# inksci/TRPO

Hardware: AMD Instinct MI355X
Metric: TRPO updates/sec (10-iter CG + linesearch) at N states; FVP GB/s vs HBM peak (higher is better)
Workload: dtype fp32 (f16x3 split); 1 GPU; C4: 8M states, obs 128, 256x256 tanh MLP, 18 actions; full update = discount+standardise+pg+10 CG+shs FVP+line search+final losses; n_states=8000000, obs_dim=128, n_actions=18, num_params=103442, cg_iters=10, parallelism=dp1 (row shards, RCCL all-reduce of [P] FVP/grad + loss scalars)

## Files before the change

trpo_amd/csrc/kernels.h:

```cpp
#pragma once
#include <hip/hip_runtime.h>
#include <cstdint>

namespace trpo {

struct Options {
  int split_mfma;
  int split_wg;
  int chain;
  int split_f16;
  int split_min_k;
  int graphs;
  int tail;
  int fused;
  int low_seg;
  int planes;
  int rbwd0;
  int hbwd2;
  int head_fwd;
  int splits;
  int pg_splits;
  int ls_fused;
  int cg_fuse_reduce;
  int cg_p_img;
  int rfwd01;
  int fwd01;
  int rh1_planes;
  int rbwd0_bdma;
};

constexpr int kAmaxSub = 256, kAmaxStride = 32, kAmaxSlot = kAmaxSub * kAmaxStride;

__host__ __device__ inline int f16_scale_exp(float m) {
  if (!(m > 0.0f) || !(m < 3.0e38f)) return 0;
  int q = 0;
  (void)frexpf(m, &q);
  int e = 12 - q;
  return e < -100 ? -100 : (e > 100 ? 100 : e);
}
extern Options g_options;
int* option_slot(const char* name);

struct GemmSeg {
  const float* A;
  const float* B;
  int lda, ldb, K;
  const uint16_t* B3 = nullptr;
  int ldk = 0, plane = 0;
  const unsigned* amaxA = nullptr;
  const unsigned* amaxB = nullptr;
  const uint16_t* Ah = nullptr;
  const uint16_t* Al = nullptr;
  int ldp = 0, mpad = 0;
  const int* eAp = nullptr;
  const uint16_t* Bb = nullptr;
};

enum class RowEpi : int {
  kTanh = 0,
  kRHidden = 1,
  kPrepBwd = 2,
// ... 600 lines not shown
```

trpo_amd/csrc/options.cpp:

```cpp
#include "kernels.h"

#include <cstdlib>
#include <cstring>

namespace trpo {
namespace {

struct OptionRow {
  const char* name;
  const char* env;
  int Options::*field;
  int dflt;
};
constexpr OptionRow kOptionRows[] = {
    {"split_mfma", "TRPO_SPLIT_MFMA", &Options::split_mfma, 5},
    {"split_wg", "TRPO_SPLIT_WG", &Options::split_wg, 1},
    {"chain", "TRPO_CHAIN", &Options::chain, 1},
    {"split_f16", "TRPO_SPLIT_F16", &Options::split_f16, 1},
    {"split_min_k", "TRPO_SPLIT_MIN_K", &Options::split_min_k, 0},
    {"graphs", "TRPO_GRAPHS", &Options::graphs, 1},
    {"tail", "TRPO_TAIL", &Options::tail, 1},
    {"fused", "TRPO_FUSED", &Options::fused, 3},
    {"low_seg", "TRPO_LOW_SEG", &Options::low_seg, 14},
    {"planes", "TRPO_PLANES", &Options::planes, 1},
    {"rbwd0", "TRPO_RBWD0", &Options::rbwd0, 1},
    {"hbwd2", "TRPO_HBWD2", &Options::hbwd2, 2},
    {"head_fwd", "TRPO_HEAD_FWD", &Options::head_fwd, 1},
    {"splits", "TRPO_SPLITS", &Options::splits, 0},
    {"pg_splits", "TRPO_PG_SPLITS", &Options::pg_splits, 0},
    {"ls_fused", "TRPO_LS_FUSED", &Options::ls_fused, 1},
    {"cg_fuse_reduce", "TRPO_CG_FUSE_REDUCE", &Options::cg_fuse_reduce, 1},
    {"cg_p_img", "TRPO_CG_P_IMG", &Options::cg_p_img, 1},
    {"rfwd01", "TRPO_RFWD01", &Options::rfwd01, 1},
    {"fwd01", "TRPO_FWD01", &Options::fwd01, 1},
    {"rh1_planes", "TRPO_RH1_PLANES", &Options::rh1_planes, 1},
    {"rbwd0_bdma", "TRPO_RBWD0_BDMA", &Options::rbwd0_bdma, 1},
};
static_assert(sizeof kOptionRows / sizeof kOptionRows[0] == sizeof(Options) / sizeof(int),
              "every field of Options needs a row");

Options options_from_env() {
  Options o{};
  for (const OptionRow& r : kOptionRows) {
    const char* e = std::getenv(r.env);
    o.*r.field = e ? std::atoi(e) : r.dflt;
  }
  return o;
}

}

Options g_options = options_from_env();

int* option_slot(const char* name) {
  for (const OptionRow& r : kOptionRows)
    if (!std::strcmp(name, r.name)) return &(g_options.*r.field);
  return nullptr;
}

}
```

trpo_amd/csrc/rfwd.hip:

```cpp
#include "chain_common.h"

#include <stdexcept>
#include <type_traits>

namespace trpo {
namespace {

#ifndef RF_SGB
#define RF_SGB 1
#endif
#ifndef RF_ILV
#define RF_ILV 1
#endif
#ifndef RF_HOIST
#define RF_HOIST 0
#endif
#ifndef RF_HEAD
#define RF_HEAD 3
#endif
#ifndef RF_CSB
#define RF_CSB 1
#endif
#ifndef RF_ABL
#define RF_ABL 0
#endif

constexpr int kRfUnits = 2048;
constexpr int kRfChunks = 24;
constexpr int kRfLd = 256;
constexpr int kRfTile = 128, kRfWaves = 4;

__global__ void __launch_bounds__(256) rfwd01_img_kernel(const float* __restrict__ theta, const float* __restrict__ v,
                                                         int64_t offV0, int64_t offW1, int obs,
                                                         const unsigned* am_v0, const unsigned* am_w1,
                                                         const unsigned* am_v1, uint16_t* __restrict__ img,
                                                         const int* skip) {
  if (skip && *skip) return;
  const int eV0 = amax_exp(am_v0), eW = amax_exp(am_w1), eV = amax_exp(am_v1);
  const int gid = blockIdx.x * 256 + threadIdx.x;
  const int t = gid / 2560, rem = gid % 2560;
  if (t >= 8) return;
  float x[8];
  u32x4* dst;
  int plane_units;
  float sc;
  if (rem < 512) {
    const int f = rem >> 4, u = rem & 15, ks = u >> 1, h = u & 1;
#pragma unroll
    for (int q = 0; q < 8; ++q) {
      const int k = 16 * ks + 8 * h + q;
      x[q] = k < obs ? v[offV0 + (int64_t)k * 256 + 32 * t + f] : 0.0f;
    }
    sc = __builtin_ldexpf(1.0f, eV0);
    dst = reinterpret_cast<u32x4*>(img) + (size_t)(3 * t) * kRfUnits + f * 16 + (u ^ (f & 15));
    plane_units = 512;
  } else {
    const int b = rem - 512, nh = b >> 10, m = (b >> 9) & 1, r = (b >> 2) & 127, u = b & 3, uu = u >> 1, h = u & 1;
    const float* src = m ? v : theta;
#pragma unroll
    for (int q = 0; q < 8; ++q) {
      const int k = 32 * t + 16 * uu + 4 * h + 8 * (q >> 2) + (q & 3);
      x[q] = src[offW1 + (int64_t)k * 256 + 128 * nh + r];
    }
    sc = __builtin_ldexpf(1.0f, m ? eV : eW);
    dst = reinterpret_cast<u32x4*>(img) + (size_t)(3 * t + 1 + nh) * kRfUnits + m * 1024 + r * 4 +
          (u ^ ((r >> 2) & 3));
    plane_units = 512;
  }
  f16x8 hi, lo;
  split8(x, sc, hi, lo);
  dst[0] = __builtin_bit_cast(u32x4, hi);
  dst[plane_units] = __builtin_bit_cast(u32x4, lo);
}

__device__ __forceinline__ void rf_dma16(__amdgpu_buffer_rsrc_t rsrc, unsigned voff, unsigned soff, unsigned lds) {
  unsigned keep;
  asm volatile("s_mov_b32 %0, m0\n\ts_mov_b32 m0, %3\n\ts_nop 0\n\tbuffer_load_dwordx4 %1, %2, 0 offen lds\n\t"
               "s_mov_b32 m0, %0"
               : "=&s"(keep)
               : "v"(voff + soff), "s"(rsrc), "s"(lds));
}

template <int KS0, bool PL>
__global__ void __launch_bounds__(kRfWaves * 64, 1) rfwd01_kernel(const Rfwd01Args a) {
  static_assert(!RF_ILV || KS0 == 8, "interleaved DMA: one instruction per k-step of phase A");
  __shared__ u32x4 q0[kRfUnits], q1[kRfUnits], q2[kRfUnits], q3[kRfUnits];
  __shared__ float cvec[2][256];
  __shared__ float red[3][16];
  __shared__ int pex[kRfWaves][32];
  if (a.skip && *a.skip) return;
  const int tid = threadIdx.x, lane = tid & 63, s = lane & 31, h = lane >> 5;
  const int wv = __builtin_amdgcn_readfirstlane(tid >> 6);
  const int eX = __builtin_amdgcn_readfirstlane(*a.eX);
  const int eV0 = __builtin_amdgcn_readfirstlane(amax_exp(a.am_v0));
  const int eW = __builtin_amdgcn_readfirstlane(amax_exp(a.am_w1));
  const int eV = __builtin_amdgcn_readfirstlane(amax_exp(a.am_v1));
  const float uA = __builtin_ldexpf(1.0f, -(eX + eV0));
  const int64_t ntiles = (a.n + kRfTile - 1) / kRfTile;
  const __amdgpu_buffer_rsrc_t rimg =
      __builtin_amdgcn_make_buffer_rsrc((void*)a.img, 0, kRfChunks * kRfUnits * 16, 0x00020000);
  const __amdgpu_buffer_rsrc_t rxh = __builtin_amdgcn_make_buffer_rsrc((void*)a.Xh, 0, 0x7ffffff0, 0x00020000);
  const __amdgpu_buffer_rsrc_t rxl = __builtin_amdgcn_make_buffer_rsrc((void*)a.Xl, 0, 0x7ffffff0, 0x00020000);
  for (int i = tid; i < 256; i += kRfWaves * 64) {
    cvec[0][i] = a.c0[i];
    cvec[1][i] = a.c1[i];
  }
  float nv0 = 0.0f, mc0 = 0.0f;
  if constexpr (RF_CSB) {
    float q = 0.0f;
    for (int k = 0; k < a.obs; ++k) {
      const float x = a.V0[(int64_t)k * 256 + tid];
      q = fmaf(x, x, q);
    }
    float m1 = max32_dpp(sqrtf(q)), m2 = max32_dpp(fabsf(a.c0[tid]));
    m1 = fmaxf(m1, __shfl_xor(m1, 32));
    m2 = fmaxf(m2, __shfl_xor(m2, 32));
    if (lane == 0) {
      red[0][wv] = m1;
      red[1][wv] = m2;
    }
    __syncthreads();
    nv0 = fmaxf(fmaxf(red[0][0], red[0][1]), fmaxf(red[0][2], red[0][3]));
    mc0 = fmaxf(fmaxf(red[1][0], red[1][1]), fmaxf(red[1][2], red[1][3]));
    __syncthreads();
  }
  int eR = 0;
  if constexpr (PL) {
    static_assert(RF_CSB, "the planes' exponent comes from the bound");
    const float bnd = sqrtf((float)a.obs) * __builtin_ldexpf(1.0f, 12 - eX) * nv0 * 1.01f + mc0;
    eR = __builtin_amdgcn_readfirstlane(f16_scale_exp(bnd));
    if (blockIdx.x == 0 && tid == 0) *a.e_rh1 = eR;
// ... 23 lines not shown
#pragma unroll
    for (int i = 0; i < 8; ++i) dma_one(A, c, sl, r0w, i);
  };
  using kA = std::true_type;
  using kB = std::false_type;
  auto arrive = [&](bool far, bool first_a0) __attribute__((always_inline)) {
    __builtin_amdgcn_sched_barrier(0);
    if (far) asm volatile("s_waitcnt vmcnt(63)" ::: "memory");
    else if (first_a0 || (RF_ABL & 8) != 0) asm volatile("s_waitcnt vmcnt(16)" ::: "memory");
    else asm volatile("s_waitcnt vmcnt(20)" ::: "memory");
    lds_barrier();
  };
  const unsigned xlane = (unsigned)(s * 32 + 8 * h) * 2u;
  auto xload = [&](int64_t row0, f16x8 (&x)[KS0][2]) __attribute__((always_inline)) {
    if constexpr ((RF_ABL & 16) != 0) {
#pragma unroll
      for (int ks = 0; ks < KS0; ++ks) {
        unsigned u = (unsigned)row0 + ks;
        asm volatile("" : "+v"(u));
        x[ks][0] = x[ks][1] = __builtin_bit_cast(f16x8, u32x4{u, u, u, u});
      }
      return;
    }
#pragma unroll
    for (int ks = 0; ks < KS0; ++ks) {
      const int so = (int)((((unsigned)(ks >> 1) * (unsigned)a.x_mpad + (unsigned)row0) * 32u + 16u * (ks & 1)) * 2u);
      x[ks][0] = __builtin_bit_cast(f16x8, __builtin_amdgcn_raw_buffer_load_b128(rxh, xlane, so, 0));
      x[ks][1] = __builtin_bit_cast(f16x8, __builtin_amdgcn_raw_buffer_load_b128(rxl, xlane, so, 0));
    }
  };
  const unsigned hlane = PL ? (unsigned)((s >> 1) * kPairLd + 16 * (s & 1) + 4 * h) * 4u
                            : (unsigned)(s * kRfLd + 4 * h) * 4u;

  f16x8 xt[KS0][2];
  xload((int64_t)blockIdx.x * kRfTile + wv * 32, xt);
  __builtin_amdgcn_s_waitcnt(0x0f70);
  {
    const int64_t r0f = (int64_t)blockIdx.x * kRfTile + wv * 32;
    dma(kA{}, 0, 0, r0f);
    dma(kB{}, 1, 1, r0f);
    dma(kB{}, 2, 2, r0f);
  }

  float mR = 0.0f, mZ = 0.0f;
  for (int64_t tile = blockIdx.x; tile < ntiles; tile += gridDim.x) {
    const bool first = tile == (int64_t)blockIdx.x;
    const int64_t r0 = tile * kRfTile + wv * 32;
    const int64_t r0n = r0 + (int64_t)gridDim.x * kRfTile;
    const int rows = rows_of(r0);
    const __amdgpu_buffer_rsrc_t rrh =
        __builtin_amdgcn_make_buffer_rsrc((void*)(a.RH1 + r0 * kRfLd), 0, PL ? 0 : rows * kRfLd * 4, 0x00020000);
    f32x16 acc[8];
#pragma unroll
    for (int i = 0; i < 8; ++i) acc[i] = f32x16{};
    int Ps = 0;
    if constexpr (RF_CSB) {
      float q = 0.0f;
#pragma unroll
      for (int ks = 0; ks < KS0; ++ks) {
        const f16x8 x8 = xt[ks][0];
        q = __builtin_amdgcn_fdot2(__builtin_shufflevector(x8, x8, 0, 1), __builtin_shufflevector(x8, x8, 0, 1), q, false);
        q = __builtin_amdgcn_fdot2(__builtin_shufflevector(x8, x8, 2, 3), __builtin_shufflevector(x8, x8, 2, 3), q, false);
        q = __builtin_amdgcn_fdot2(__builtin_shufflevector(x8, x8, 4, 5), __builtin_shufflevector(x8, x8, 4, 5), q, false);
        q = __builtin_amdgcn_fdot2(__builtin_shufflevector(x8, x8, 6, 7), __builtin_shufflevector(x8, x8, 6, 7), q, false);
      }
      q = xadd_f<true>(q);
      const float bnd = __builtin_ldexpf(sqrtf(q), -eX) * nv0 * 1.01f + mc0;
      Ps = min(bnd > 0.0f ? f16_scale_exp(bnd) + eW : 1000, f16_scale_exp(1.0f) + eV);
    }
    int* px = pex[wv];
#pragma unroll 1
    for (int tq = 0; tq < 2; ++tq) {
#pragma unroll
      for (int tt = 0; tt < 4; ++tt) {
        const int t = 4 * tq + tt;
        const int cA = 3 * t, sA = (3 * tt) % 4;
        const bool far = t == 0 && !first;
// ... 140 lines not shown
            if (RF_SGB && (RF_ABL & 3) == 0 && k + 1 < 8) {
              __builtin_amdgcn_sched_group_barrier(0x100, 4, 0);
              __builtin_amdgcn_sched_group_barrier(0x008, 6, 0);
            }
          }
          __builtin_amdgcn_sched_barrier(0);
        }
      }
    }
    xload(r0n < a.x_mpad ? r0n : 0, xt);
    if (h == 0) px[s] = Ps;
    __builtin_amdgcn_wave_barrier();
    __builtin_amdgcn_fence(__ATOMIC_SEQ_CST, "wavefront");
    float un[16];
#pragma unroll
    for (int r = 0; r < 16; ++r) un[r] = __builtin_ldexpf(1.0f, -px[8 * (r >> 2) + 4 * h + (r & 3)]);
    __builtin_amdgcn_wave_barrier();
    const __amdgpu_buffer_rsrc_t rz =
        __builtin_amdgcn_make_buffer_rsrc((void*)(a.RZ2 + r0 * kRfLd), 0, rows * kRfLd * 4, 0x00020000);
    const unsigned zlane = (unsigned)(4 * h * kRfLd + s) * 4u;
#pragma unroll
    for (int tn = 0; tn < 8; ++tn) {
      const float cn = cvec[1][32 * tn + s];
#pragma unroll
      for (int r = 0; r < 16; ++r) {
        const float o = acc[tn][r] * un[r] + cn;
        mZ = fmaxf(mZ, fabsf(o));
        if constexpr ((RF_ABL & 8) == 0)
          __builtin_amdgcn_raw_buffer_store_b32(__builtin_bit_cast(unsigned, o), rz, zlane,
                                                ((8 * (r >> 2) + (r & 3)) * kRfLd + 32 * tn) * 4, 0);
      }
    }
  }
  asm volatile("s_waitcnt vmcnt(0)" ::: "memory");
  if constexpr (PL) {
    if ((a.n & 1) != 0 && (int64_t)blockIdx.x == (ntiles - 1) % (int64_t)gridDim.x) {
      __syncthreads();
      int col = threadIdx.x;
      asm volatile("" : "+v"(col));
      unsigned short* const p = reinterpret_cast<unsigned short*>(a.RH1 + (a.n >> 1) * kPairLd + col) + 1;
      p[0] = 0;
      p[2 * pair_plane_dwords(a.n)] = 0;
    }
  }
  amax_commit3<true>(a.am_rh1, mR, a.am_rz2, mZ, nullptr, 0.0f, red);
}


constexpr int kFwChunks = 16;

__global__ void __launch_bounds__(256) fwd01_img_kernel(const float* __restrict__ th, int64_t offW0, int64_t offW1,
                                                        int obs, const unsigned* am_w0, const unsigned* am_w1,
                                                        uint16_t* __restrict__ img) {
  const int eW0 = amax_exp(am_w0), eW1 = amax_exp(am_w1);
  const int gid = blockIdx.x * 256 + threadIdx.x;
  const int t = gid / 1536, rem = gid % 1536;
  if (t >= 8) return;
  float x[8];
  u32x4* dst;
  int plane_units;
  float sc;
  if (rem < 512) {
    const int f = rem >> 4, u = rem & 15, ks = u >> 1, h = u & 1;
#pragma unroll
    for (int q = 0; q < 8; ++q) {
      const int k = 16 * ks + 8 * h + q;
      x[q] = k < obs ? th[offW0 + (int64_t)k * 256 + 32 * t + f] : 0.0f;
    }
    sc = __builtin_ldexpf(1.0f, eW0);
    dst = reinterpret_cast<u32x4*>(img) + (size_t)(2 * t) * kRfUnits + f * 16 + (u ^ (f & 15));
    plane_units = 512;
  } else {
    const int b = rem - 512, r = b >> 2, u = b & 3, uu = u >> 1, h = u & 1;
#pragma unroll
    for (int q = 0; q < 8; ++q) {
      const int k = 32 * t + 16 * uu + 4 * h + 8 * (q >> 2) + (q & 3);
      x[q] = th[offW1 + (int64_t)k * 256 + r];
    }
    sc = __builtin_ldexpf(1.0f, eW1);
    dst = reinterpret_cast<u32x4*>(img) + (size_t)(2 * t + 1) * kRfUnits + r * 4 + (u ^ ((r >> 2) & 3));
    plane_units = 1024;
  }
  f16x8 hi, lo;
  split8(x, sc, hi, lo);
  dst[0] = __builtin_bit_cast(u32x4, hi);
  dst[plane_units] = __builtin_bit_cast(u32x4, lo);
}

template <int KS0, bool PREP>
__global__ void __launch_bounds__(kRfWaves * 64, 1) fwd01_kernel(const Fwd01Args a) {
  __shared__ u32x4 q0[kRfUnits], q1[kRfUnits], q2[kRfUnits], q3[kRfUnits];
  __shared__ float cvec[2][256];
  const int tid = threadIdx.x, lane = tid & 63, s = lane & 31, h = lane >> 5;
  const int wv = __builtin_amdgcn_readfirstlane(tid >> 6);
  const int eX = __builtin_amdgcn_readfirstlane(*a.eX);
  const int eW0 = __builtin_amdgcn_readfirstlane(amax_exp(a.am_w0));
  const int eW1 = __builtin_amdgcn_readfirstlane(amax_exp(a.am_w1));
  const float uA = __builtin_ldexpf(1.0f, -(eX + eW0));
  const int P = f16_scale_exp(1.0f) + eW1;
  const float sH = __builtin_ldexpf(1.0f, P - eW1), uP = __builtin_ldexpf(1.0f, -P);
  const int64_t ntiles = (a.n + kRfTile - 1) / kRfTile;
  const __amdgpu_buffer_rsrc_t rimg =
      __builtin_amdgcn_make_buffer_rsrc((void*)a.img, 0, kFwChunks * kRfUnits * 16, 0x00020000);
  const __amdgpu_buffer_rsrc_t rxh = __builtin_amdgcn_make_buffer_rsrc((void*)a.Xh, 0, 0x7ffffff0, 0x00020000);
  const __amdgpu_buffer_rsrc_t rxl = __builtin_amdgcn_make_buffer_rsrc((void*)a.Xl, 0, 0x7ffffff0, 0x00020000);
  for (int i = tid; i < 256; i += kRfWaves * 64) {
    cvec[0][i] = a.b0[i];
    cvec[1][i] = a.b1[i];
  }
  asm volatile("s_waitcnt vmcnt(0)" ::: "memory");
  auto slot = [&](int k) -> u32x4* { return k == 0 ? q0 : k == 1 ? q1 : k == 2 ? q2 : q3; };
  auto rows_of = [&](int64_t r0w) { return (int)(a.n - r0w < 32 ? (a.n - r0w > 0 ? a.n - r0w : 0) : 32); };
  auto dma_one = [&](int c, int sl, int i) __attribute__((always_inline)) {
    const unsigned lds0 = (unsigned)(uintptr_t)slot(sl);
    const int base = wv * 64 + i * kRfWaves * 64;
    rf_dma16(rimg, (unsigned)(base + lane) * 16u, (unsigned)c * kRfUnits * 16u, lds0 + (unsigned)base * 16u);
  };
  constexpr int S = PREP ? 4 : 0;
  auto arrive = [&](int cnt) __attribute__((always_inline)) {
    __builtin_amdgcn_sched_barrier(0);
    if (cnt >= 63) asm volatile("s_waitcnt vmcnt(63)" ::: "memory");
    else if (PREP && cnt == 20) asm volatile("s_waitcnt vmcnt(20)" ::: "memory");
    else if (PREP && cnt == 16) asm volatile("s_waitcnt vmcnt(16)" ::: "memory");
    else asm volatile("s_waitcnt vmcnt(12)" ::: "memory");
    lds_barrier();
  };
  const unsigned xlane = (unsigned)(s * 32 + 8 * h) * 2u;
  auto xload = [&](int64_t row0, f16x8 (&x)[KS0][2]) __attribute__((always_inline)) {
#pragma unroll
    for (int ks = 0; ks < KS0; ++ks) {
      const int so = (int)((((unsigned)(ks >> 1) * (unsigned)a.x_mpad + (unsigned)row0) * 32u + 16u * (ks & 1)) * 2u);
      x[ks][0] = __builtin_bit_cast(f16x8, __builtin_amdgcn_raw_buffer_load_b128(rxh, xlane, so, 0));
      x[ks][1] = __builtin_bit_cast(f16x8, __builtin_amdgcn_raw_buffer_load_b128(rxl, xlane, so, 0));
    }
  };
  const unsigned hlane = (unsigned)(s * kRfLd + 4 * h) * 4u;

  f16x8 xt[KS0][2];
  xload((int64_t)blockIdx.x * kRfTile + wv * 32, xt);
  __builtin_amdgcn_s_waitcnt(0x0f70);
#pragma unroll
  for (int i = 0; i < 4; ++i) dma_one(0, 0, i);
#pragma unroll
  for (int i = 0; i < 8; ++i) dma_one(1, 1, i);
#pragma unroll
  for (int i = 0; i < 4; ++i) dma_one(2, 2, i);

  for (int64_t tile = blockIdx.x; tile < ntiles; tile += gridDim.x) {
    const bool first = tile == (int64_t)blockIdx.x;
    const int64_t r0 = tile * kRfTile + wv * 32;
    const int64_t r0n = r0 + (int64_t)gridDim.x * kRfTile;
    const int rows = rows_of(r0);
    f32x16 acc[8];
#pragma unroll
    for (int i = 0; i < 8; ++i) acc[i] = f32x16{};
#pragma unroll 1
    for (int tq = 0; tq < 2; ++tq) {
#pragma unroll
      for (int tt = 0; tt < 4; ++tt) {
// ... 47 lines not shown
          const int bu = col * 4 + ((2 * ((k >> 2) & 1) + h) ^ ((col >> 2) & 3));
          f[0] = __builtin_bit_cast(f16x8, B[bu]);
          f[1] = __builtin_bit_cast(f16x8, B[1024 + bu]);
        };
        ldb(0, fb[0]);
#pragma unroll
        for (int k = 0; k < 16; ++k) {
          __builtin_amdgcn_sched_barrier(0);
          if (k < 4) dma_one(cB3, (sB + 3) % 4, k);
          if (k + 1 < 16) ldb(k + 1, fb[(k + 1) & 1]);
          const int uu = (k >> 2) & 1, tn = k & 3, nh = k >> 3;
          acc[4 * nh + tn] = mfma3(aH[uu][0], aH[uu][1], fb[k & 1][0], fb[k & 1][1], acc[4 * nh + tn]);
          if (RF_SGB && k + 1 < 16) {
            __builtin_amdgcn_sched_group_barrier(0x100, 2, 0);
            __builtin_amdgcn_sched_group_barrier(0x008, 3, 0);
          }
        }
        __builtin_amdgcn_sched_barrier(0);
      }
    }
    xload(r0n < a.x_mpad ? r0n : 0, xt);
    const __amdgpu_buffer_rsrc_t rz =
        __builtin_amdgcn_make_buffer_rsrc((void*)(a.H2 + r0 * kRfLd), 0, rows * kRfLd * 4, 0x00020000);
    const unsigned zlane = (unsigned)(4 * h * kRfLd + s) * 4u;
#pragma unroll
    for (int tn = 0; tn < 8; ++tn) {
      const float bn = cvec[1][32 * tn + s];
#pragma unroll
      for (int r = 0; r < 16; ++r)
        __builtin_amdgcn_raw_buffer_store_b32(__builtin_bit_cast(unsigned, tanh_fast(acc[tn][r] * uP + bn)), rz,
                                              zlane, ((8 * (r >> 2) + (r & 3)) * kRfLd + 32 * tn) * 4, 0);
    }
  }
  asm volatile("s_waitcnt vmcnt(0)" ::: "memory");
}

}

bool rfwd01_eligible(int L, const int* w, const int* wp) {
  return L == 3 && w[0] >= 1 && w[0] <= 128 && w[1] == 256 && w[2] == 256 && wp[1] == 256 && wp[2] == 256;
}

size_t rfwd01_img_bytes() { return (size_t)kRfChunks * kRfUnits * 16; }

void launch_rfwd01_img(const float* theta, const float* v, int64_t offV0, int64_t offW1, int obs,
                       const unsigned* am_v0, const unsigned* am_w1, const unsigned* am_v1, uint16_t* img,
                       const int* skip, hipStream_t s) {
  hipLaunchKernelGGL(rfwd01_img_kernel, dim3(8 * 2560 / 256), dim3(256), 0, s, theta, v, offV0, offW1, obs, am_v0,
                     am_w1, am_v1, img, skip);
}

void launch_rfwd01(const Rfwd01Args& a, int num_cus, hipStream_t s) {
  if (a.n <= 0) return;
  if (a.obs < 1 || a.obs > 128 || a.ldh != 256 || a.ldz != 256)
    throw std::runtime_error("rfwd01: unsupported shape");
  if (!rfwd01_rows_ok(a.x_mpad) || a.x_mpad < (a.n + kRfTile - 1) / kRfTile * kRfTile)
    throw std::runtime_error("rfwd01: X plane geometry");
  const int64_t ntiles = (a.n + kRfTile - 1) / kRfTile;
  const int grid = (int)std::min<int64_t>(ntiles, (int64_t)num_cus);
  if (a.e_rh1) {
    if (!pair_planes_rows_ok(a.x_mpad)) throw std::runtime_error("rfwd01: RH1 plane geometry");
    hipLaunchKernelGGL((rfwd01_kernel<8, true>), dim3(grid), dim3(kRfWaves * 64), 0, s, a);
  } else {
    hipLaunchKernelGGL((rfwd01_kernel<8, false>), dim3(grid), dim3(kRfWaves * 64), 0, s, a);
  }
}

bool fwd01_eligible(int L, const int* w, const int* wp) { return rfwd01_eligible(L, w, wp); }

size_t fwd01_img_bytes() { return (size_t)kFwChunks * kRfUnits * 16; }

void launch_fwd01_img(const float* th, int64_t offW0, int64_t offW1, int obs, const unsigned* am_w0,
                      const unsigned* am_w1, uint16_t* img, hipStream_t s) {
  hipLaunchKernelGGL(fwd01_img_kernel, dim3(8 * 1536 / 256), dim3(256), 0, s, th, offW0, offW1, obs, am_w0, am_w1,
                     img);
}

void launch_fwd01(const Fwd01Args& a, int num_cus, hipStream_t s) {
  if (a.n <= 0) return;
  if (a.obs < 1 || a.obs > 128) throw std::runtime_error("fwd01: unsupported shape");
  if (!rfwd01_rows_ok(a.x_mpad) || a.x_mpad < (a.n + kRfTile - 1) / kRfTile * kRfTile)
    throw std::runtime_error("fwd01: X plane geometry");
  const int64_t ntiles = (a.n + kRfTile - 1) / kRfTile;
  const int grid = (int)std::min<int64_t>(ntiles, (int64_t)num_cus);
  if (a.H1) hipLaunchKernelGGL((fwd01_kernel<8, true>), dim3(grid), dim3(kRfWaves * 64), 0, s, a);
  else hipLaunchKernelGGL((fwd01_kernel<8, false>), dim3(grid), dim3(kRfWaves * 64), 0, s, a);
}

}
```

Baseline: 2.613 updates/s.

## Add 256-state tile variants of rfwd01 and fwd01 kernels, on by default

Adds an HV=2 path to the fused R-op forward and forward layer-0/1 kernels, so each wave processes 64 states (two 32-row halves) per tile instead of 32. Each weight chunk staged into LDS is then reused across twice as many states, which halves weight DMA traffic per state and amortises LDS reads over more MFMAs. The change also adds a new LDS ring, new inline-asm MFMA helpers and a new DMA schedule. In exchange it roughly doubles accumulator registers, raises LDS use, and makes the tail tiles coarser. It is selected by a new rf_tile option that defaults to 256.

```diff
diff --git a/trpo_amd/csrc/kernels.h b/trpo_amd/csrc/kernels.h
--- a/trpo_amd/csrc/kernels.h
+++ b/trpo_amd/csrc/kernels.h
@@ -27,6 +27,7 @@
   int fwd01;
   int rh1_planes;
   int rbwd0_bdma;
+  int rf_tile;
 };
 
 constexpr int kAmaxSub = 256, kAmaxStride = 32, kAmaxSlot = kAmaxSub * kAmaxStride;
diff --git a/trpo_amd/csrc/options.cpp b/trpo_amd/csrc/options.cpp
--- a/trpo_amd/csrc/options.cpp
+++ b/trpo_amd/csrc/options.cpp
@@ -35,6 +35,7 @@
     {"fwd01", "TRPO_FWD01", &Options::fwd01, 1},
     {"rh1_planes", "TRPO_RH1_PLANES", &Options::rh1_planes, 1},
     {"rbwd0_bdma", "TRPO_RBWD0_BDMA", &Options::rbwd0_bdma, 1},
+    {"rf_tile", "TRPO_RF_TILE", &Options::rf_tile, 256},
 };
 static_assert(sizeof kOptionRows / sizeof kOptionRows[0] == sizeof(Options) / sizeof(int),
               "every field of Options needs a row");
diff --git a/trpo_amd/csrc/rfwd.hip b/trpo_amd/csrc/rfwd.hip
--- a/trpo_amd/csrc/rfwd.hip
+++ b/trpo_amd/csrc/rfwd.hip
@@ -29,6 +29,7 @@
 constexpr int kRfChunks = 24;
 constexpr int kRfLd = 256;
 constexpr int kRfTile = 128, kRfWaves = 4;
+constexpr bool kRf256 = RF_CSB && RF_ILV && RF_ABL == 0;
 
 __global__ void __launch_bounds__(256) rfwd01_img_kernel(const float* __restrict__ theta, const float* __restrict__ v,
                                                          int64_t offV0, int64_t offW1, int obs,
@@ -81,13 +82,47 @@
                : "v"(voff + soff), "s"(rsrc), "s"(lds));
 }
 
-template <int KS0, bool PL>
+typedef const u32x4 __attribute__((address_space(3))) lds_u32x4;
+__device__ __forceinline__ f16x8 lds_f16x8(unsigned addr, int off_bytes) {
+  return __builtin_bit_cast(f16x8, *reinterpret_cast<lds_u32x4*>((uintptr_t)addr + off_bytes));
+}
+__device__ __forceinline__ unsigned opaque_v(unsigned x) {
+  asm volatile("" : "+v"(x));
+  return x;
+}
+__device__ __forceinline__ void rf_dma16s(__amdgpu_buffer_rsrc_t rsrc, unsigned voff, unsigned soff, unsigned lds) {
+  unsigned keep;
+  asm volatile("s_mov_b32 %0, m0\n\ts_mov_b32 m0, %4\n\ts_nop 0\n\tbuffer_load_dwordx4 %1, %2, %3 offen lds\n\t"
+               "s_mov_b32 m0, %0"
+               : "=&s"(keep)
+               : "v"(voff), "s"(rsrc), "s"(soff), "s"(lds));
+}
+
+__device__ __forceinline__ void mfma3_v(const f16x8& ah, const f16x8& al, const f16x8& bh, const f16x8& bl, f32x16& c) {
+  asm("v_mfma_f32_32x32x16_f16 %0, %1, %2, %0\n\t"
+      "v_mfma_f32_32x32x16_f16 %0, %3, %4, %0\n\t"
+      "v_mfma_f32_32x32x16_f16 %0, %3, %2, %0"
+      : "+v"(c)
+      : "v"(al), "v"(bh), "v"(ah), "v"(bl));
+}
+__device__ __forceinline__ void mfma3_v0(const f16x8& ah, const f16x8& al, const f16x8& bh, const f16x8& bl, f32x16& c) {
+  asm("v_mfma_f32_32x32x16_f16 %0, %1, %2, 0\n\t"
+      "v_mfma_f32_32x32x16_f16 %0, %3, %4, %0\n\t"
+      "v_mfma_f32_32x32x16_f16 %0, %3, %2, %0"
+      : "=&v"(c)
+      : "v"(al), "v"(bh), "v"(ah), "v"(bl));
+}
+__device__ __forceinline__ void mfma_v_done(f32x16& c) { asm("s_nop 15\n\ts_nop 7" : "+v"(c)); }
+
+template <int KS0, bool PL, int HV = 1>
 __global__ void __launch_bounds__(kRfWaves * 64, 1) rfwd01_kernel(const Rfwd01Args a) {
   static_assert(!RF_ILV || KS0 == 8, "interleaved DMA: one instruction per k-step of phase A");
   __shared__ u32x4 q0[kRfUnits], q1[kRfUnits], q2[kRfUnits], q3[kRfUnits];
   __shared__ float cvec[2][256];
   __shared__ float red[3][16];
-  __shared__ int pex[kRfWaves][32];
+  __shared__ int pex[kRfWaves][32 * HV];
+  __shared__ __attribute__((aligned(1024))) u32x4 ring2[HV == 1 ? 1 : 7 * kRfUnits / 2];
+  constexpr int kTile = 128 * HV;
   if (a.skip && *a.skip) return;
   const int tid = threadIdx.x, lane = tid & 63, s = lane & 31, h = lane >> 5;
   const int wv = __builtin_amdgcn_readfirstlane(tid >> 6);
@@ -96,7 +131,7 @@
   const int eW = __builtin_amdgcn_readfirstlane(amax_exp(a.am_w1));
   const int eV = __builtin_amdgcn_readfirstlane(amax_exp(a.am_v1));
   const float uA = __builtin_ldexpf(1.0f, -(eX + eV0));
-  const int64_t ntiles = (a.n + kRfTile - 1) / kRfTile;
+  const int64_t ntiles = (a.n + kTile - 1) / kTile;
   const __amdgpu_buffer_rsrc_t rimg =
       __builtin_amdgcn_make_buffer_rsrc((void*)a.img, 0, kRfChunks * kRfUnits * 16, 0x00020000);
   const __amdgpu_buffer_rsrc_t rxh = __builtin_amdgcn_make_buffer_rsrc((void*)a.Xh, 0, 0x7ffffff0, 0x00020000);
@@ -186,6 +221,246 @@
   const unsigned hlane = PL ? (unsigned)((s >> 1) * kPairLd + 16 * (s & 1) + 4 * h) * 4u
                             : (unsigned)(s * kRfLd + 4 * h) * 4u;
 
+  float mR = 0.0f, mZ = 0.0f;
+  if constexpr (HV == 2) {
+    static_assert(KS0 == 8 && kRf256, "the 256-state tiles exist in the default form only");
+    const unsigned lds0 = (unsigned)(uintptr_t)ring2;
+    unsigned ln = (unsigned)lane;
+    const float nv0s = __builtin_bit_cast(float, __builtin_amdgcn_readfirstlane(__builtin_bit_cast(int, nv0)));
+    const float mc0s = __builtin_bit_cast(float, __builtin_amdgcn_readfirstlane(__builtin_bit_cast(int, mc0)));
+    constexpr unsigned kSlotB = 3 * kRfUnits / 2 * 16;
+    auto dma_a = [&](int t2, int64_t r0w, int i) __attribute__((always_inline)) {
+      if (i < 4) {
+        rf_dma16s(rimg, (unsigned)(wv * 64 + ln) * 16u, (unsigned)(3 * t2 * kRfUnits + i * 256) * 16u,
+                  lds0 + (unsigned)(wv * 64 + i * 256) * 16u);
+      } else {
+        const int ih = i - 4;
+        const int64_t left = a.n - r0w;
+        const int rw = (int)(left < 64 ? (left > 0 ? left : 0) : 64);
+        const __amdgpu_buffer_rsrc_t rh =
+            __builtin_amdgcn_make_buffer_rsrc((void*)(a.H1 + r0w * kRfLd), 0, rw * kRfLd * 4, 0x00020000);
+        const unsigned vh0 = (ln >> 3) * (unsigned)(kRfLd * 4) + 16u * ((ln & 7) ^ (ln >> 4));
+        rf_dma16s(rh, (vh0 ^ (unsigned)(64 * (ih & 1))) + (unsigned)(8 * ih * kRfLd) * 4u,
+                  (unsigned)(32 * t2) * 4u, lds0 + (unsigned)(1024 + wv * 512 + 64 * ih) * 16u);
+      }
+    };
+    auto dma_b = [&](int t2, int nh, int i) __attribute__((always_inline)) {
+      rf_dma16s(rimg, (unsigned)(wv * 64 + ln) * 16u, (unsigned)((3 * t2 + 1 + nh) * kRfUnits + i * 256) * 16u,
+                lds0 + kSlotB + (unsigned)(nh * kRfUnits + wv * 64 + i * 256) * 16u);
+    };
+    auto arrive2 = [&](int cnt) __attribute__((always_inline)) {
+      __builtin_amdgcn_sched_barrier(0);
+      if (cnt >= 63) asm volatile("s_waitcnt vmcnt(63)" ::: "memory");
+      else if (cnt == 16) asm volatile("s_waitcnt vmcnt(16)" ::: "memory");
+      else asm volatile("s_waitcnt vmcnt(8)" ::: "memory");
+      lds_barrier();
+    };
+    auto xload2 = [&](int64_t row0, f16x8 (&x)[KS0][2]) __attribute__((always_inline)) {
+      const unsigned xl = ((ln & 31) * 32 + 8 * (ln >> 5)) * 2u;
+#pragma unroll
+      for (int ks = 0; ks < KS0; ++ks) {
+        const int so = (int)((((unsigned)(ks >> 1) * (unsigned)a.x_mpad + (unsigned)row0) * 32u + 16u * (ks & 1)) * 2u);
+        x[ks][0] = __builtin_bit_cast(f16x8, __builtin_amdgcn_raw_buffer_load_b128(rxh, xl, so, 0));
+        x[ks][1] = __builtin_bit_cast(f16x8, __builtin_amdgcn_raw_buffer_load_b128(rxl, xl, so, 0));
+      }
+    };
+    f16x8 xt[2][KS0][2];
+    const int64_t r0f = (int64_t)blockIdx.x * kTile + wv * 64;
+#pragma unroll
+    for (int hf = 0; hf < 2; ++hf) xload2(r0f + 32 * hf, xt[hf]);
+    __builtin_amdgcn_s_waitcnt(0x0f70);
+#pragma unroll
+    for (int i = 0; i < 12; ++i) dma_a(0, r0f, i);
+#pragma unroll
+    for (int i = 0; i < 8; ++i) dma_b(0, 0, i);
+
+    for (int64_t tile = blockIdx.x; tile < ntiles; tile += gridDim.x) {
+      const bool first = tile == (int64_t)blockIdx.x;
+      const int64_t r0 = tile * kTile + wv * 64;
+      const int64_t r0n = r0 + (int64_t)gridDim.x * kTile;
+      f32x16 acc[2][8];
+      int Ps[2];
+#pragma unroll
+      for (int hf = 0; hf < 2; ++hf) {
+#pragma unroll
+        for (int i = 0; i < 8; ++i) acc[hf][i] = f32x16{};
+        float q = 0.0f;
+#pragma unroll
+        for (int ks = 0; ks < KS0; ++ks) {
+          const f16x8 x8 = xt[hf][ks][0];
+          q = __builtin_amdgcn_fdot2(__builtin_shufflevector(x8, x8, 0, 1), __builtin_shufflevector(x8, x8, 0, 1), q, false);
+          q = __builtin_amdgcn_fdot2(__builtin_shufflevector(x8, x8, 2, 3), __builtin_shufflevector(x8, x8, 2, 3), q, false);
+          q = __builtin_amdgcn_fdot2(__builtin_shufflevector(x8, x8, 4, 5), __builtin_shufflevector(x8, x8, 4, 5), q, false);
+          q = __builtin_amdgcn_fdot2(__builtin_shufflevector(x8, x8, 6, 7), __builtin_shufflevector(x8, x8, 6, 7), q, false);
+        }
+        q = xadd_f<true>(q);
+        const float bnd = __builtin_ldexpf(sqrtf(q), -eX) * nv0s * 1.01f + mc0s;
+        Ps[hf] = min(bnd > 0.0f ? f16_scale_exp(bnd) + eW : 1000, f16_scale_exp(1.0f) + eV);
+      }
+      int* px = pex[wv];
+#pragma unroll 1
+      for (int t = 0; t < 8; ++t) {
+        const bool far = t == 0 && !first;
+        ln = opaque_v(ln);
+        const unsigned s = ln & 31, h = ln >> 5;
+        const bool odd = (s & 1) != 0;
+        const unsigned hlane = PL ? ((s >> 1) * kPairLd + 16 * (s & 1) + 4 * h) * 4u : (s * kRfLd + 4 * h) * 4u;
+        const int t1 = t + 1 < 8 ? t + 1 : 0;
+        const int64_t r1 = t + 1 < 8 ? r0 : r0n;
+        arrive2(far ? 63 : 8);
+        f16x8 aR[2][2][2], aH[2][2][2];
+#pragma unroll
+        for (int hf = 0; hf < 2; ++hf) {
+          const unsigned abase = lds0 + (s * 16 + (h ^ (s & 15))) * 16u;
+          f32x16 accA;
+          f16x8 fa[2][2];
+          auto lda = [&](int ks, f16x8 (&f)[2]) __attribute__((always_inline)) {
+            f[0] = lds_f16x8(abase ^ (unsigned)(32 * ks), 0);
+            f[1] = lds_f16x8(abase ^ (unsigned)(32 * ks), 512 * 16);
+          };
+          lda(0, fa[0]);
+#pragma unroll
+          for (int ks = 0; ks < KS0; ++ks) {
+            __builtin_amdgcn_sched_barrier(0);
+            if ((ks & 1) == 0) dma_b(t, 1, 4 * hf + (ks >> 1));
+            if (ks + 1 < KS0) lda(ks + 1, fa[(ks + 1) & 1]);
+            if (ks == 0) mfma3_v0(fa[0][0], fa[0][1], xt[hf][0][0], xt[hf][0][1], accA);
+            else mfma3_v(fa[ks & 1][0], fa[ks & 1][1], xt[hf][ks][0], xt[hf][ks][1], accA);
+          }
+          mfma_v_done(accA);
+          __builtin_amdgcn_sched_barrier(0);
+          const unsigned hbase = lds0 + (1024 + wv * 512 + s * 8 + (h ^ ((s >> 1) & 7))) * 16u;
+          const float* const cb = &cvec[0][32 * t + 4 * h];
+          const int rows = rows_of(r0 + 32 * hf);
+          const __amdgpu_buffer_rsrc_t rrh = __builtin_amdgcn_make_buffer_rsrc(
+              (void*)(a.RH1 + (r0 + 32 * hf) * kRfLd), 0, PL ? 0 : rows * kRfLd * 4, 0x00020000);
+          const float sR = __builtin_ldexpf(1.0f, Ps[hf] - eW), sH = __builtin_ldexpf(1.0f, Ps[hf] - eV);
+          float rh[16], hv[16];
+          float mt = 0.0f;
+#pragma unroll
+          for (int uu = 0; uu < 2; ++uu) {
+#pragma unroll
+            for (int j = 2 * uu; j < 2 * uu + 2; ++j) {
+              const f32x4 v4 = __builtin_bit_cast(f32x4, lds_f16x8(hbase ^ (unsigned)(32 * j), hf * 256 * 16));
+#pragma unroll
+              for (int i = 0; i < 4; ++i) {
+                const int r = 4 * j + i;
+                hv[r] = v4[i];
+                rh[r] = one_minus_sq(hv[r]) * (accA[r] * uA + cb[8 * j + i]);
+                mt = fmaxf(mt, fabsf(rh[r]));
+              }
+              if constexpr (!PL)
+                __builtin_amdgcn_raw_buffer_store_b128(
+                    __builtin_bit_cast(u32x4, f32x4{rh[4 * j], rh[4 * j + 1], rh[4 * j + 2], rh[4 * j + 3]}), rrh,
+                    hlane, (32 * t + 8 * j) * 4, 0);
+            }
+            split8(rh + 8 * uu, sR, aR[hf][uu][0], aR[hf][uu][1]);
+            split8(hv + 8 * uu, sH, aH[hf][uu][0], aH[hf][uu][1]);
+            __builtin_amdgcn_sched_barrier(0);
+          }
+          if constexpr (PL) {
+            float* const ph = a.RH1 + ((r0 + 32 * hf) >> 1) * kPairLd;
+            int pbytes = (rows + 1) / 2 * kPairLd * 4;
+            asm volatile("" : "+s"(pbytes));
+            const __amdgpu_buffer_rsrc_t rph = __builtin_amdgcn_make_buffer_rsrc((void*)ph, 0, pbytes, 0x00020000);
+            const __amdgpu_buffer_rsrc_t rpl =
+                __builtin_amdgcn_make_buffer_rsrc((void*)(ph + plane_lo), 0, pbytes, 0x00020000);
+#pragma unroll
+            for (int j = 0; j < 2; ++j) {
+              u32x4 Hq, Lq;
+#pragma unroll
+              for (int q = 0; q < 4; ++q) {
+                const int i = 4 * j + q;
+                const float nl = dpp_f<kDppX1>(rh[i]), nh = dpp_f<kDppX1>(rh[8 + i]);
+                const float ev = (odd ? nh : rh[i]) * scR, od = (odd ? rh[8 + i] : nl) * scR;
+                const u32x2 p = split2(ev, od);
+                Hq[q] = p[0];
+                Lq[q] = p[1];
+              }
+              __builtin_amdgcn_raw_buffer_store_b128(Hq, rph, hlane, (32 * t + 8 * j) * 4, 0);
+              __builtin_amdgcn_raw_buffer_store_b128(Lq, rpl, hlane, (32 * t + 8 * j) * 4, 0);
+              __builtin_amdgcn_sched_barrier(0);
+            }
+          }
+          mR = fmaxf(mR, mt);
+          __builtin_amdgcn_sched_barrier(0);
+        }
+#pragma unroll
+        for (int nh = 0; nh < 2; ++nh) {
+          arrive2(far && nh == 0 ? 63 : 16);
+          const unsigned bbase = lds0 + kSlotB + (s * 4 + (h ^ ((s >> 2) & 3))) * 16u;
+          f16x8 fb[2][4];
+          auto ldb = [&](int k, f16x8 (&f)[4]) __attribute__((always_inline)) {
+            const unsigned ad = bbase ^ (unsigned)(32 * (k >> 2));
+            const int off = (nh * kRfUnits + 32 * (k & 3) * 4) * 16;
+            f[0] = lds_f16x8(ad, off);
+            f[1] = lds_f16x8(ad, off + 512 * 16);
+            f[2] = lds_f16x8(ad, off + 1024 * 16);
+            f[3] = lds_f16x8(ad, off + 1536 * 16);
+          };
+          ldb(0, fb[0]);
+#pragma unroll
+          for (int k = 0; k < 8; ++k) {
+            __builtin_amdgcn_sched_barrier(0);
+            if (nh == 0) {
+              dma_a(t1, r1, k);
+              if (k < 4) dma_a(t1, r1, 8 + k);
+            } else {
+              dma_b(t1, 0, k);
+            }
+            if (k + 1 < 8) ldb(k + 1, fb[(k + 1) & 1]);
+            const int uu = k >> 2, tn = k & 3;
+            const f16x8(&f)[4] = fb[k & 1];
+#pragma unroll
+            for (int hf = 0; hf < 2; ++hf) {
+              f32x16 c = acc[hf][4 * nh + tn];
+              c = mfma3(aR[hf][uu][0], aR[hf][uu][1], f[0], f[1], c);
+              c = mfma3(aH[hf][uu][0], aH[hf][uu][1], f[2], f[3], c);
+              acc[hf][4 * nh + tn] = c;
+            }
+            if (RF_SGB && k + 1 < 8) {
+              __builtin_amdgcn_sched_group_barrier(0x100, 4, 0);
+              __builtin_amdgcn_sched_group_barrier(0x008, 12, 0);
+            }
+          }
+          __builtin_amdgcn_sched_barrier(0);
+        }
+      }
+      ln = opaque_v(ln);
+#pragma unroll
+      for (int hf = 0; hf < 2; ++hf) xload2(r0n < a.x_mpad ? r0n + 32 * hf : 0, xt[hf]);
+      const unsigned s = ln & 31, h = ln >> 5;
+      if (h == 0) {
+        px[s] = Ps[0];
+        px[32 + s] = Ps[1];
+      }
+      __builtin_amdgcn_wave_barrier();
+      __builtin_amdgcn_fence(__ATOMIC_SEQ_CST, "wavefront");
+      const unsigned zlane = (4 * h * kRfLd + s) * 4u;
+#pragma unroll
+      for (int hf = 0; hf < 2; ++hf) {
+        float un[16];
+#pragma unroll
+        for (int r = 0; r < 16; ++r) un[r] = __builtin_ldexpf(1.0f, -px[32 * hf + 8 * (r >> 2) + 4 * h + (r & 3)]);
+        const __amdgpu_buffer_rsrc_t rz = __builtin_amdgcn_make_buffer_rsrc(
+            (void*)(a.RZ2 + (r0 + 32 * hf) * kRfLd), 0, rows_of(r0 + 32 * hf) * kRfLd * 4, 0x00020000);
+#pragma unroll
+        for (int tn = 0; tn < 8; ++tn) {
+          const float cn = cvec[1][32 * tn + s];
+          asm volatile("" : "+a"(acc[hf][tn]));
+#pragma unroll
+          for (int r = 0; r < 16; ++r) {
+            const float o = acc[hf][tn][r] * un[r] + cn;
+            mZ = fmaxf(mZ, fabsf(o));
+            __builtin_amdgcn_raw_buffer_store_b32(__builtin_bit_cast(unsigned, o), rz, zlane,
+                                                  ((8 * (r >> 2) + (r & 3)) * kRfLd + 32 * tn) * 4, 0);
+          }
+        }
+      }
+      __builtin_amdgcn_wave_barrier();
+    }
+  }
+  if constexpr (HV == 1) {
   f16x8 xt[KS0][2];
   xload((int64_t)blockIdx.x * kRfTile + wv * 32, xt);
   __builtin_amdgcn_s_waitcnt(0x0f70);
@@ -196,7 +471,6 @@
     dma(kB{}, 2, 2, r0f);
   }
 
-  float mR = 0.0f, mZ = 0.0f;
   for (int64_t tile = blockIdx.x; tile < ntiles; tile += gridDim.x) {
     const bool first = tile == (int64_t)blockIdx.x;
     const int64_t r0 = tile * kRfTile + wv * 32;
@@ -403,6 +677,7 @@
       }
     }
   }
+  }
   asm volatile("s_waitcnt vmcnt(0)" ::: "memory");
   if constexpr (PL) {
     if ((a.n & 1) != 0 && (int64_t)blockIdx.x == (ntiles - 1) % (int64_t)gridDim.x) {
@@ -458,9 +733,10 @@
   dst[plane_units] = __builtin_bit_cast(u32x4, lo);
 }
 
-template <int KS0, bool PREP>
+template <int KS0, bool PREP, int HV = 1>
 __global__ void __launch_bounds__(kRfWaves * 64, 1) fwd01_kernel(const Fwd01Args a) {
   __shared__ u32x4 q0[kRfUnits], q1[kRfUnits], q2[kRfUnits], q3[kRfUnits];
+  __shared__ __attribute__((aligned(1024))) u32x4 ring2[HV == 1 ? 1 : 4 * kRfUnits];
   __shared__ float cvec[2][256];
   const int tid = threadIdx.x, lane = tid & 63, s = lane & 31, h = lane >> 5;
   const int wv = __builtin_amdgcn_readfirstlane(tid >> 6);
@@ -470,7 +746,8 @@
   const float uA = __builtin_ldexpf(1.0f, -(eX + eW0));
   const int P = f16_scale_exp(1.0f) + eW1;
   const float sH = __builtin_ldexpf(1.0f, P - eW1), uP = __builtin_ldexpf(1.0f, -P);
-  const int64_t ntiles = (a.n + kRfTile - 1) / kRfTile;
+  constexpr int kTile = 128 * HV, kWS = 32 * HV;
+  const int64_t ntiles = (a.n + kTile - 1) / kTile;
   const __amdgpu_buffer_rsrc_t rimg =
       __builtin_amdgcn_make_buffer_rsrc((void*)a.img, 0, kFwChunks * kRfUnits * 16, 0x00020000);
   const __amdgpu_buffer_rsrc_t rxh = __builtin_amdgcn_make_buffer_rsrc((void*)a.Xh, 0, 0x7ffffff0, 0x00020000);
@@ -480,22 +757,165 @@
     cvec[1][i] = a.b1[i];
   }
   asm volatile("s_waitcnt vmcnt(0)" ::: "memory");
-  auto slot = [&](int k) -> u32x4* { return k == 0 ? q0 : k == 1 ? q1 : k == 2 ? q2 : q3; };
+  auto slot = [&](int k) -> u32x4* {
+    if constexpr (HV != 1) return ring2 + k * kRfUnits;
+    return k == 0 ? q0 : k == 1 ? q1 : k == 2 ? q2 : q3;
+  };
   auto rows_of = [&](int64_t r0w) { return (int)(a.n - r0w < 32 ? (a.n - r0w > 0 ? a.n - r0w : 0) : 32); };
   auto dma_one = [&](int c, int sl, int i) __attribute__((always_inline)) {
     const unsigned lds0 = (unsigned)(uintptr_t)slot(sl);
     const int base = wv * 64 + i * kRfWaves * 64;
-    rf_dma16(rimg, (unsigned)(base + lane) * 16u, (unsigned)c * kRfUnits * 16u, lds0 + (unsigned)base * 16u);
+    if constexpr (HV == 1)
+      rf_dma16(rimg, (unsigned)(base + lane) * 16u, (unsigned)c * kRfUnits * 16u, lds0 + (unsigned)base * 16u);
+    else
+      rf_dma16s(rimg, (unsigned)tid * 16u, (unsigned)(c * kRfUnits + i * kRfWaves * 64) * 16u,
+                lds0 + (unsigned)base * 16u);
   };
   constexpr int S = PREP ? 4 : 0;
+  constexpr int kCntA = HV == 1 ? 12 + S : 12 + 2 * S, kCntB = HV == 1 ? 12 + 2 * S : 12 + 3 * S;
+  constexpr int kCntB0 = HV == 1 ? 12 + S : 12 + 2 * S;
   auto arrive = [&](int cnt) __attribute__((always_inline)) {
     __builtin_amdgcn_sched_barrier(0);
     if (cnt >= 63) asm volatile("s_waitcnt vmcnt(63)" ::: "memory");
+    else if (HV != 1 && PREP && cnt == 24) asm volatile("s_waitcnt vmcnt(24)" ::: "memory");
     else if (PREP && cnt == 20) asm volatile("s_waitcnt vmcnt(20)" ::: "memory");
     else if (PREP && cnt == 16) asm volatile("s_waitcnt vmcnt(16)" ::: "memory");
     else asm volatile("s_waitcnt vmcnt(12)" ::: "memory");
     lds_barrier();
   };
+  if constexpr (HV == 2) {
+  const unsigned xlane = (unsigned)(s * 32 + 8 * h) * 2u;
+  auto xload = [&](int64_t row0, f16x8 (&x)[KS0][2]) __attribute__((always_inline)) {
+#pragma unroll
+    for (int ks = 0; ks < KS0; ++ks) {
+      const int so = (int)((((unsigned)(ks >> 1) * (unsigned)a.x_mpad + (unsigned)row0) * 32u + 16u * (ks & 1)) * 2u);
+      x[ks][0] = __builtin_bit_cast(f16x8, __builtin_amdgcn_raw_buffer_load_b128(rxh, xlane, so, 0));
+      x[ks][1] = __builtin_bit_cast(f16x8, __builtin_amdgcn_raw_buffer_load_b128(rxl, xlane, so, 0));
+    }
+  };
+  const unsigned hlane = (unsigned)(s * kRfLd + 4 * h) * 4u;
+
+  f16x8 xt[HV][KS0][2];
+#pragma unroll
+  for (int hf = 0; hf < HV; ++hf) xload((int64_t)blockIdx.x * kTile + wv * kWS + 32 * hf, xt[hf]);
+  __builtin_amdgcn_s_waitcnt(0x0f70);
+#pragma unroll
+  for (int i = 0; i < 4; ++i) dma_one(0, 0, i);
+#pragma unroll
+  for (int i = 0; i < 8; ++i) dma_one(1, 1, i);
+#pragma unroll
+  for (int i = 0; i < 4; ++i) dma_one(2, 2, i);
+
+  for (int64_t tile = blockIdx.x; tile < ntiles; tile += gridDim.x) {
+    const bool first = tile == (int64_t)blockIdx.x;
+    const int64_t r0 = tile * kTile + wv * kWS;
+    const int64_t r0n = r0 + (int64_t)gridDim.x * kTile;
+    int rows[HV];
+#pragma unroll
+    for (int hf = 0; hf < HV; ++hf) rows[hf] = rows_of(r0 + 32 * hf);
+    f32x16 acc[HV][8];
+#pragma unroll
+    for (int hf = 0; hf < HV; ++hf)
+#pragma unroll
+      for (int i = 0; i < 8; ++i) acc[hf][i] = f32x16{};
+#pragma unroll 1
+    for (int tq = 0; tq < 2; ++tq) {
+#pragma unroll
+      for (int tt = 0; tt < 4; ++tt) {
+        const int t = 4 * tq + tt;
+        const int cA = 2 * t, sA = (2 * tt) % 4, cB = cA + 1, sB = (2 * tt + 1) % 4;
+        arrive(!first && t <= 1 ? 63 : (first && t == 0 ? 12 : kCntA));
+        const int cA3 = cA + 3 < kFwChunks ? cA + 3 : cA + 3 - kFwChunks;
+        const u32x4* SA = slot(sA);
+        f16x8 aH[HV][2][2];
+#pragma unroll
+        for (int hf = 0; hf < HV; ++hf) {
+        f32x16 accA;
+        f16x8 fa[2][2];
+        const unsigned abase = opaque_v((unsigned)(uintptr_t)SA + (unsigned)(s * 16 + (h ^ (s & 15))) * 16u);
+        auto lda = [&](int ks, f16x8 (&f)[2]) __attribute__((always_inline)) {
+          f[0] = lds_f16x8(abase ^ (unsigned)(32 * ks), 0);
+          f[1] = lds_f16x8(abase ^ (unsigned)(32 * ks), 512 * 16);
+        };
+        lda(0, fa[0]);
+#pragma unroll
+        for (int ks = 0; ks < KS0; ++ks) {
+          __builtin_amdgcn_sched_barrier(0);
+          if ((ks & 1) == 0) dma_one(cA3, (sA + 3) % 4, 4 * hf + (ks >> 1));
+          if (ks + 1 < KS0) lda(ks + 1, fa[(ks + 1) & 1]);
+          if (ks == 0) mfma3_v0(fa[0][0], fa[0][1], xt[hf][0][0], xt[hf][0][1], accA);
+          else mfma3_v(fa[ks & 1][0], fa[ks & 1][1], xt[hf][ks][0], xt[hf][ks][1], accA);
+        }
+        mfma_v_done(accA);
+        __builtin_amdgcn_sched_barrier(0);
+        float hv[16];
+#pragma unroll
+        for (int r = 0; r < 16; ++r)
+          hv[r] = tanh_fast(accA[r] * uA + cvec[0][32 * t + 8 * (r >> 2) + 4 * h + (r & 3)]);
+        if constexpr (PREP) {
+          const __amdgpu_buffer_rsrc_t rh1 = __builtin_amdgcn_make_buffer_rsrc(
+              (void*)(a.H1 + (r0 + 32 * hf) * kRfLd), 0, rows[hf] * kRfLd * 4, 0x00020000);
+#pragma unroll
+          for (int j = 0; j < 4; ++j)
+            __builtin_amdgcn_raw_buffer_store_b128(
+                __builtin_bit_cast(u32x4, f32x4{hv[4 * j], hv[4 * j + 1], hv[4 * j + 2], hv[4 * j + 3]}), rh1,
+                hlane, (32 * t + 8 * j) * 4, 0);
+        }
+#pragma unroll
+        for (int uu = 0; uu < 2; ++uu) split8(hv + 8 * uu, sH, aH[hf][uu][0], aH[hf][uu][1]);
+        }
+        arrive(!first && t == 0 ? 63 : (first && t == 0 ? kCntB0 : kCntB));
+        const int cB3 = cB + 3 < kFwChunks ? cB + 3 : cB + 3 - kFwChunks;
+        const u32x4* B = slot(sB);
+        f16x8 fb[2][2];
+        const unsigned bbase = opaque_v((unsigned)(uintptr_t)B + (unsigned)(s * 4 + (h ^ ((s >> 2) & 3))) * 16u);
+        auto ldb = [&](int k, f16x8 (&f)[2]) __attribute__((always_inline)) {
+          const unsigned ad = bbase ^ (unsigned)(32 * ((k >> 2) & 1));
+          const int off = (128 * (k >> 3) + 32 * (k & 3)) * 4 * 16;
+          f[0] = lds_f16x8(ad, off);
+          f[1] = lds_f16x8(ad, off + 1024 * 16);
+        };
+        ldb(0, fb[0]);
+#pragma unroll
+        for (int k = 0; k < 16; ++k) {
+          __builtin_amdgcn_sched_barrier(0);
+          if (k < 4) dma_one(cB3, (sB + 3) % 4, k);
+          if (k + 1 < 16) ldb(k + 1, fb[(k + 1) & 1]);
+          const int uu = (k >> 2) & 1, tn = k & 3, nh = k >> 3;
+#pragma unroll
+          for (int hf = 0; hf < HV; ++hf)
+            acc[hf][4 * nh + tn] =
+                mfma3(aH[hf][uu][0], aH[hf][uu][1], fb[k & 1][0], fb[k & 1][1], acc[hf][4 * nh + tn]);
+          if (RF_SGB && k + 1 < 16) {
+            __builtin_amdgcn_sched_group_barrier(0x100, 2, 0);
+            __builtin_amdgcn_sched_group_barrier(0x008, 3 * HV, 0);
+          }
+        }
+        __builtin_amdgcn_sched_barrier(0);
+      }
+    }
+#pragma unroll
+    for (int hf = 0; hf < HV; ++hf) xload(r0n < a.x_mpad ? r0n + 32 * hf : 0, xt[hf]);
+#pragma unroll
+    for (int hf = 0; hf < HV; ++hf) {
+    const __amdgpu_buffer_rsrc_t rz =
+        __builtin_amdgcn_make_buffer_rsrc((void*)(a.H2 + (r0 + 32 * hf) * kRfLd), 0, rows[hf] * kRfLd * 4, 0x00020000);
+    const unsigned zlane = (unsigned)(4 * h * kRfLd + s) * 4u;
+#pragma unroll
+    for (int tn = 0; tn < 8; ++tn) {
+      const float bn = cvec[1][32 * tn + s];
+      asm volatile("" : "+a"(acc[hf][tn]));
+#pragma unroll
+      for (int r = 0; r < 16; ++r) {
+        __builtin_amdgcn_raw_buffer_store_b32(__builtin_bit_cast(unsigned, tanh_fast(acc[hf][tn][r] * uP + bn)), rz,
+                                              zlane, ((8 * (r >> 2) + (r & 3)) * kRfLd + 32 * tn) * 4, 0);
+        if ((r & 3) == 3) __builtin_amdgcn_sched_barrier(0);
+      }
+    }
+    }
+  }
+  }
+  if constexpr (HV == 1) {
   const unsigned xlane = (unsigned)(s * 32 + 8 * h) * 2u;
   auto xload = [&](int64_t row0, f16x8 (&x)[KS0][2]) __attribute__((always_inline)) {
 #pragma unroll
@@ -609,9 +1029,16 @@
                                               zlane, ((8 * (r >> 2) + (r & 3)) * kRfLd + 32 * tn) * 4, 0);
     }
   }
+  }
   asm volatile("s_waitcnt vmcnt(0)" ::: "memory");
 }
 
+}
+
+static int rf_tile_states() {
+  const int t = g_options.rf_tile;
+  if (t != 128 && t != 256) throw std::runtime_error("rf_tile: 128 or 256");
+  return t;
 }
 
 bool rfwd01_eligible(int L, const int* w, const int* wp) {
@@ -631,12 +1058,20 @@
   if (a.n <= 0) return;
   if (a.obs < 1 || a.obs > 128 || a.ldh != 256 || a.ldz != 256)
     throw std::runtime_error("rfwd01: unsupported shape");
-  if (!rfwd01_rows_ok(a.x_mpad) || a.x_mpad < (a.n + kRfTile - 1) / kRfTile * kRfTile)
+  const int tile = rf_tile_states();
+  if (!rfwd01_rows_ok(a.x_mpad) || a.x_mpad < (a.n + tile - 1) / tile * tile)
     throw std::runtime_error("rfwd01: X plane geometry");
-  const int64_t ntiles = (a.n + kRfTile - 1) / kRfTile;
+  const int64_t ntiles = (a.n + tile - 1) / tile;
   const int grid = (int)std::min<int64_t>(ntiles, (int64_t)num_cus);
-  if (a.e_rh1) {
-    if (!pair_planes_rows_ok(a.x_mpad)) throw std::runtime_error("rfwd01: RH1 plane geometry");
+  if (a.e_rh1 && !pair_planes_rows_ok(a.x_mpad)) throw std::runtime_error("rfwd01: RH1 plane geometry");
+  if (tile == 256) {
+    if constexpr (kRf256) {
+      if (a.e_rh1) hipLaunchKernelGGL((rfwd01_kernel<8, true, 2>), dim3(grid), dim3(kRfWaves * 64), 0, s, a);
+      else hipLaunchKernelGGL((rfwd01_kernel<8, false, 2>), dim3(grid), dim3(kRfWaves * 64), 0, s, a);
+    } else {
+      throw std::runtime_error("rfwd01: this build has no 256-state tiles (rf_tile = 128)");
+    }
+  } else if (a.e_rh1) {
     hipLaunchKernelGGL((rfwd01_kernel<8, true>), dim3(grid), dim3(kRfWaves * 64), 0, s, a);
   } else {
     hipLaunchKernelGGL((rfwd01_kernel<8, false>), dim3(grid), dim3(kRfWaves * 64), 0, s, a);
@@ -656,12 +1091,19 @@
 void launch_fwd01(const Fwd01Args& a, int num_cus, hipStream_t s) {
   if (a.n <= 0) return;
   if (a.obs < 1 || a.obs > 128) throw std::runtime_error("fwd01: unsupported shape");
-  if (!rfwd01_rows_ok(a.x_mpad) || a.x_mpad < (a.n + kRfTile - 1) / kRfTile * kRfTile)
+  const int tile = rf_tile_states();
+  if (!rfwd01_rows_ok(a.x_mpad) || a.x_mpad < (a.n + tile - 1) / tile * tile)
     throw std::runtime_error("fwd01: X plane geometry");
-  const int64_t ntiles = (a.n + kRfTile - 1) / kRfTile;
+  const int64_t ntiles = (a.n + tile - 1) / tile;
   const int grid = (int)std::min<int64_t>(ntiles, (int64_t)num_cus);
-  if (a.H1) hipLaunchKernelGGL((fwd01_kernel<8, true>), dim3(grid), dim3(kRfWaves * 64), 0, s, a);
-  else hipLaunchKernelGGL((fwd01_kernel<8, false>), dim3(grid), dim3(kRfWaves * 64), 0, s, a);
-}
-
-}
+  if (tile == 256) {
+    if (a.H1) hipLaunchKernelGGL((fwd01_kernel<8, true, 2>), dim3(grid), dim3(kRfWaves * 64), 0, s, a);
+    else hipLaunchKernelGGL((fwd01_kernel<8, false, 2>), dim3(grid), dim3(kRfWaves * 64), 0, s, a);
+  } else if (a.H1) {
+    hipLaunchKernelGGL((fwd01_kernel<8, true>), dim3(grid), dim3(kRfWaves * 64), 0, s, a);
+  } else {
+    hipLaunchKernelGGL((fwd01_kernel<8, false>), dim3(grid), dim3(kRfWaves * 64), 0, s, a);
+  }
+}
+
+}
```

Result: no change. 2.616 updates/s, median of 6 (+0.1%).
